# soon-yau/upgpt

Hardware: AMD Instinct MI355X
Metric: 256x256 images/sec, 50-step DDIM, bs=8/GPU; UNet MFMA util % (higher is better)
Workload: dtype f16; 1 GPU; BASELINE configs[1]: bs=8/GPU, 256x256 px (latent 4x32x32), 50-step DDIM eta=0, text-only cond [B,87,768], UNet(bbox.yaml) + VAE decode, EMA weights, no CFG; batch_per_gpu=8, ddim_steps=50, batches_in_flight_per_gpu=4, lane_hw_queues=measured, parallelism=replica-dp1, one all-gather of images per batch

## Files before the change

include/upk.h:

```cpp
#ifndef UPK_H_
#define UPK_H_

#include <stddef.h>
#include <stdint.h>

#ifdef __cplusplus
extern "C" {
#endif

#define UPK_VERSION 100

#define UPK_OK 0
#define UPK_EINVAL (-1)
#define UPK_ESHAPE (-2)
#define UPK_EWORKSPACE (-3)
#define UPK_EHIP (-4)
#define UPK_ENODEV (-5)

typedef struct upk_ctx upk_ctx;
typedef void* upk_stream;

int upk_version(void);
int upk_create(upk_ctx** out, int device);
int upk_destroy(upk_ctx* ctx);
// ... 121 lines not shown
  const float* vec;
  float ln_eps;
  int32_t ln_dim;
  void* t0;
  int32_t ld_t0;
  void* qk;
  int32_t ld_qk;
  void* vt;
  int32_t vt_ld;
  int32_t hw, rows_per_wg;
  const float* gn_part;
  const float* gn_gamma;
  const float* gn_beta;
  int32_t gn_nblk, gn_ld, gn_groups;
  float gn_eps;
} upk_hblock_desc;
int upk_head_block_f16(upk_ctx* ctx, const upk_hblock_desc* d, upk_stream stream);
int upk_head_block_supported(upk_ctx* ctx, const upk_hblock_desc* d);

int upk_gemm_f16(upk_ctx* ctx, const void* a, int lda, int m, int k, const void* w_packed,
                 int n_out, int n_pad, const float* bias, const void* residual, int ld_res,
                 void* y, int ldy, int flags, upk_stream stream);

int upk_conv_autotune(upk_ctx* ctx, const upk_conv_desc* d, upk_stream stream, int reps, int* best_cfg,
                      int* best_splitk, float* best_us, float* default_us);

int upk_conv_override(upk_ctx* ctx, int cfg, int splitk);
int upk_conv_num_configs(void);
const char* upk_conv_config_name(int cfg);

int upk_attention_f16(upk_ctx* ctx, const void* q, int ldq, long long q_batch_stride,
                      const void* k, int ldk, long long k_batch_stride, const void* vt, int vt_ld,
                      void* out, int ldo, long long o_batch_stride, int batch, int heads, int n_q,
                      int n_kv, int d, float scale, upk_stream stream);

int upk_attention_causal_f16(upk_ctx* ctx, const void* q, int ldq, long long q_batch_stride,
                             const void* k, int ldk, long long k_batch_stride, const void* vt, int vt_ld,
                             void* out, int ldo, long long o_batch_stride, int batch, int heads, int n,
                             int d, float scale, upk_stream stream);

int upk_attention_qproj_f16(upk_ctx* ctx, const void* x, int ldx, long long xbs, int cq, int ln_dim, float ln_eps,
                            const void* wq, const float* wq_colsum, const float* wq_bias, const void* k, int ldk,
                            long long kbs, const void* vt, int vt_ld, void* out, int ldo, long long obs, int batch,
                            int heads, int n_q, int n_kv, int d, float scale, upk_stream stream);

int upk_embed_tokens_f16(upk_ctx* ctx, const int32_t* ids, const void* tok_emb, const void* pos_emb, int rows,
                         int seq, int dim, int vocab, void* out, int ld_out, upk_stream stream);

int upk_gather_rows_f16(upk_ctx* ctx, const void* x, int ldx, const int32_t* idx, int n, int n_src, int dim,
// ... 105 lines not shown
```

upgpt_amd/_lib.py:

```python
import contextlib
import ctypes as C
import os
import threading

import torch
from ._check import require

_HERE = os.path.dirname(os.path.abspath(__file__))
LIB_PATH = os.environ.get("UPK_LIB") or os.path.join(_HERE, "libupk.so")

SYMBOLS = [
    "upk_version", "upk_create", "upk_destroy", "upk_last_error", "upk_set_workspace", "upk_num_cus",
    "upk_pack_weight_f16", "upk_packed_weight_bytes", "upk_conv2d_nhwc_f16", "upk_gemm_f16",
    "upk_conv_autotune", "upk_conv_override", "upk_conv_num_configs", "upk_conv_config_name", "upk_conv_gn_fused",
    "upk_conv_ln_rows",
    "upk_geglu_mlp_f16", "upk_geglu_mlp_supported", "upk_cross_block_f16", "upk_cross_block_supported", "upk_head_block_f16", "upk_head_block_supported",
    "upk_attention_f16", "upk_groupnorm_nhwc_f16", "upk_groupnorm_stats_nhwc_f16", "upk_groupnorm_chunks", "upk_groupnorm_apply_nhwc_f16", "upk_groupnorm_finalize_f32", "upk_groupnorm_ws_bytes",
    "upk_layernorm_f16", "upk_timestep_embed_f16",
    "upk_nchw_f32_to_nhwc_f16", "upk_nhwc_f16_to_nchw_f32", "upk_f32_to_f16", "upk_ddim_step_f32",
    "upk_ddim_step_cfg_f32", "upk_ddim_step_edit_f32", "upk_plms_step_f32", "upk_ddpm_step_f32", "upk_attention_causal_f16", "upk_attention_qproj_f16", "upk_embed_tokens_f16",
    "upk_patchify_nchw_f32_f16", "upk_vit_assemble_f16", "upk_gather_rows_f16",
    "upk_image_finish_u8", "upk_ssim_ws_bytes", "upk_ssim_u8",
    "upk_lpips_input_f16", "upk_relu_pool_nhwc_f16", "upk_lpips_ws_bytes", "upk_lpips_layer_f16",
    "upk_advance_step", "upk_step_autoadvance", "upk_kernel_launches", "upk_graph_begin", "upk_graph_end", "upk_graph_launch", "upk_graph_destroy",
    "upk_prof_enable", "upk_prof_collect",
    "upk_stream_create_cumask", "upk_stream_destroy", "upk_probe_placement", "upk_probe_clock",
]

F_SILU, F_GEGLU, F_OUT_F32, F_OUT_NCHW_F32, F_UPSAMPLE2X, F_PAD_ASYM = 0x1, 0x2, 0x4, 0x8, 0x10, 0x20
DDPM_X0, DDPM_CLIP = 0x1, 0x2
LAYOUT_NCHW, LAYOUT_NHWC = 0, 1
FINISH_SAMPLE, FINISH_INPUT, FINISH_DENORM = 0, 1, 2
# ... 53 lines not shown
        ("ln_eps", C.c_float), ("ln_dim", C.c_int32),
        ("k_ctx", C.c_void_p), ("ldk", C.c_int32), ("n_kv", C.c_int32),
        ("vt_ctx", C.c_void_p), ("vt_ld", C.c_int32), ("scale", C.c_float),
        ("y", C.c_void_p), ("ldy", C.c_int32), ("hw", C.c_int32), ("rows_per_wg", C.c_int32),
    ]


class HblockDesc(C.Structure):
    _fields_ = [
        ("x", C.c_void_p), ("ldx", C.c_int32), ("m", C.c_int32), ("c", C.c_int32), ("heads", C.c_int32), ("d", C.c_int32),
        ("w_in", C.c_void_p), ("w_qkv", C.c_void_p), ("vec", C.c_void_p), ("ln_eps", C.c_float), ("ln_dim", C.c_int32),
        ("t0", C.c_void_p), ("ld_t0", C.c_int32), ("qk", C.c_void_p), ("ld_qk", C.c_int32),
        ("vt", C.c_void_p), ("vt_ld", C.c_int32), ("hw", C.c_int32), ("rows_per_wg", C.c_int32),
        ("gn_part", C.c_void_p), ("gn_gamma", C.c_void_p), ("gn_beta", C.c_void_p),
        ("gn_nblk", C.c_int32), ("gn_ld", C.c_int32), ("gn_groups", C.c_int32), ("gn_eps", C.c_float),
    ]


_lib = None
_lib_lock = threading.Lock()


def load_library(path=None):
    global _lib
    with _lib_lock:
        if _lib is not None and path is None:
            return _lib
        p = path or LIB_PATH
        if not os.path.exists(p):
            raise RuntimeError(
# ... 14 lines not shown
            "upk_gemm_f16": (C.c_int, [vp, vp, i32, i32, i32, vp, i32, i32, vp, vp, i32, vp, i32, i32, vp]),
            "upk_conv_autotune": (C.c_int, [vp, C.POINTER(ConvDesc), vp, i32, C.POINTER(C.c_int), C.POINTER(C.c_int),
                                            C.POINTER(C.c_float), C.POINTER(C.c_float)]),
            "upk_conv_override": (C.c_int, [vp, i32, i32]),
            "upk_conv_num_configs": (C.c_int, []),
            "upk_conv_config_name": (C.c_char_p, [i32]),
            "upk_conv_ln_rows": (C.c_int, [vp, C.POINTER(ConvDesc), C.POINTER(C.c_int)]),
            "upk_geglu_mlp_f16": (C.c_int, [vp, C.POINTER(MlpDesc), vp]),
            "upk_geglu_mlp_supported": (C.c_int, [vp, C.POINTER(MlpDesc)]),
            "upk_cross_block_f16": (C.c_int, [vp, C.POINTER(XblockDesc), vp]),
            "upk_cross_block_supported": (C.c_int, [vp, C.POINTER(XblockDesc)]),
            "upk_head_block_f16": (C.c_int, [vp, C.POINTER(HblockDesc), vp]),
            "upk_head_block_supported": (C.c_int, [vp, C.POINTER(HblockDesc)]),
            "upk_attention_f16": (C.c_int, [vp, vp, i32, i64, vp, i32, i64, vp, i32, vp, i32, i64,
                                            i32, i32, i32, i32, i32, f32, vp]),
            "upk_attention_causal_f16": (C.c_int, [vp, vp, i32, i64, vp, i32, i64, vp, i32, vp, i32, i64,
                                                   i32, i32, i32, i32, f32, vp]),
            "upk_attention_qproj_f16": (C.c_int, [vp, vp, i32, i64, i32, i32, f32, vp, vp, vp, vp, i32, i64, vp, i32, vp,
                                                  i32, i64, i32, i32, i32, i32, i32, f32, vp]),
            "upk_embed_tokens_f16": (C.c_int, [vp, vp, vp, vp, i32, i32, i32, i32, vp, i32, vp]),
            "upk_gather_rows_f16": (C.c_int, [vp, vp, i32, vp, i32, i32, i32, vp, i32, vp]),
            "upk_patchify_nchw_f32_f16": (C.c_int, [vp, vp, i32, i32, i32, i32, i32, vp, i32, vp]),
            "upk_vit_assemble_f16": (C.c_int, [vp, vp, i32, vp, vp, i32, i32, i32, vp, i32, vp]),
            "upk_groupnorm_nhwc_f16": (C.c_int, [vp, vp, i32, i32, vp, i32, i32, i32, i32, i32, vp, vp,
                                                 f32, i32, vp, i32, vp, vp]),
            "upk_groupnorm_stats_nhwc_f16": (C.c_int, [vp, vp, i32, i32, vp, i32, i32, i32, i32, i32, vp, vp]),
            "upk_groupnorm_chunks": (C.c_int, [i32]),
            "upk_groupnorm_apply_nhwc_f16": (C.c_int, [vp, vp, i32, i32, vp, i32, i32, i32, i32, i32, vp, vp,
                                                       f32, i32, vp, i32, vp, i32, i32, i32, vp, i32, i32, vp]),
            "upk_conv_gn_fused": (C.c_int, [vp, C.POINTER(ConvDesc), C.POINTER(C.c_int), C.POINTER(C.c_int)]),
# ... 351 lines not shown
```

upgpt_amd/csrc/attention.hip:

```cpp
#include <stdlib.h>

#include "common.h"

namespace {

struct AttnArgs {
  const f16* q;
  const f16* k;
  const f16* vt;
  f16* o;
  int ldq, ldk, vt_ld, ldo;
  long qbs, kbs, obs;
  int heads, nq, nkv;
  float scale_log2;
  int causal;
};

__device__ __forceinline__ float raw_exp2(float x) { return __builtin_amdgcn_exp2f(x); }
__device__ __forceinline__ float max_over_key_groups(float x) {
  unsigned u = __float_as_uint(x);
  const auto a = __builtin_amdgcn_permlane32_swap(u, u, false, false);
  u = __float_as_uint(fmaxf(__uint_as_float(a[0]), __uint_as_float(a[1])));
  const auto b = __builtin_amdgcn_permlane16_swap(u, u, false, false);
  return fmaxf(__uint_as_float(b[0]), __uint_as_float(b[1]));
}
__device__ __forceinline__ float sum_over_key_groups(float x) {
  unsigned u = __float_as_uint(x);
  const auto a = __builtin_amdgcn_permlane32_swap(u, u, false, false);
  u = __float_as_uint(__uint_as_float(a[0]) + __uint_as_float(a[1]));
  const auto b = __builtin_amdgcn_permlane16_swap(u, u, false, false);
// ... 279 lines not shown
    if (!q_ok[u]) continue;
    f16* orow = a.o + b * a.obs + (long)(q0 + u * 16 + c) * a.ldo + h * D + g * 4;
#pragma unroll
    for (int i = 0; i < DT; ++i) {
      f16x4 ov;
#pragma unroll
      for (int r = 0; r < 4; ++r) ov[r] = (f16)(o[u][i][r] * inv);
      *(f16x4*)(orow + i * 16) = ov;
    }
  }
}

constexpr int ATT_VROW = 72;
__device__ __forceinline__ int att_swz(int row, int chunk) { return chunk ^ ((-(row >> 2)) & 3); }

template <int D, int QT>
__global__ __launch_bounds__(256) void attn_lds_kernel(const AttnArgs a) {
  constexpr int KD = D / 32;
  constexpr int DT = D / 16;
  __shared__ __attribute__((aligned(16))) f16 sk[2][KD * 64 * 32];
  __shared__ __attribute__((aligned(16))) f16 sv[2][D * ATT_VROW];
  const int tid = threadIdx.x;
  const int lane = tid & 63, wave = tid >> 6;
  const int g = lane >> 4, c = lane & 15;
  const int bh = blockIdx.x;
#ifndef UPK_NO_XCD_SAMPLE
  const int nb_ = gridDim.x / a.heads;
  const int b = bh % nb_;
  const int h = bh / nb_;
#else
  const int b = bh / a.heads;
// ... 4 lines not shown

  bool q_ok[QT];
  f16x8 qf[QT][KD];
  f32x4 o[QT][DT];
  float mrun[QT];
  f32x4 lsum[QT];
#pragma unroll
  for (int u = 0; u < QT; ++u) {
    const int qi = q0 + u * 16 + c;
    q_ok[u] = qi < a.nq;
    const f16* qrow = a.q + b * a.qbs + (long)(q_ok[u] ? qi : 0) * a.ldq + h * D + g * 8;
#pragma unroll
    for (int kd = 0; kd < KD; ++kd) qf[u][kd] = q_ok[u] ? *(const f16x8*)(qrow + kd * 32) : zero8;
#pragma unroll
    for (int i = 0; i < DT; ++i) o[u][i] = (f32x4){0.f, 0.f, 0.f, 0.f};
    mrun[u] = -INFINITY;
    lsum[u] = (f32x4){0.f, 0.f, 0.f, 0.f};
  }
  const f16* ksrc = a.k + b * a.kbs + (long)(tid >> 2) * a.ldk + h * D + (tid & 3) * 8;
  const f16* vsrc = a.vt + ((long)(b * a.heads + h) * D + (tid >> 3)) * a.vt_ld + (tid & 7) * 8;
  const int kdst = (tid >> 2) * 32 + att_swz(tid >> 2, tid & 3) * 8;
  const int vdst = (tid >> 3) * ATT_VROW + (tid & 7) * 8;
  f16x8 kreg[KD], vreg[KD];
  auto fetch = [&](int kb) {
#pragma unroll
    for (int it = 0; it < KD; ++it) {
      kreg[it] = *(const f16x8*)(ksrc + (long)kb * a.ldk + it * 32);
      vreg[it] = *(const f16x8*)(vsrc + (long)it * 32 * a.vt_ld + kb);
    }
  };
  auto stash = [&](int buf) {
// ... 4 lines not shown
    }
  };
  const int ntiles = a.nkv >> 6;
  fetch(0);
  stash(0);
  __syncthreads();
  const float cs = a.scale_log2;
  const int kfrag = c * 32 + att_swz(c, g) * 8;
  for (int t = 0; t < ntiles; ++t) {
    const int buf = t & 1;
    if (t + 1 < ntiles) fetch((t + 1) << 6);
    f32x4 sc[QT][4];
#pragma unroll
    for (int tt = 0; tt < 4; ++tt)
#pragma unroll
      for (int u = 0; u < QT; ++u) sc[u][tt] = (f32x4){0.f, 0.f, 0.f, 0.f};
#pragma unroll
    for (int kd = 0; kd < KD; ++kd)
#pragma unroll
      for (int tt = 0; tt < 4; ++tt) {
        const f16x8 kf = *(const f16x8*)(&sk[buf][(kd * 64 + tt * 16) * 32 + kfrag]);
#pragma unroll
        for (int u = 0; u < QT; ++u) sc[u][tt] = __builtin_amdgcn_mfma_f32_16x16x32_f16(kf, qf[u][kd], sc[u][tt], 0, 0, 0);
      }
    f16x8 pf[QT][2];
#pragma unroll
    for (int u = 0; u < QT; ++u) {
      float mx = -INFINITY;
#pragma unroll
      for (int tt = 0; tt < 4; ++tt)
        mx = fmaxf(mx, fmaxf(fmaxf(sc[u][tt][0], sc[u][tt][1]), fmaxf(sc[u][tt][2], sc[u][tt][3])));
      mx = max_over_key_groups(mx);
      const float mnew = fmaxf(mrun[u], mx);
      if (__builtin_amdgcn_ballot_w64(mnew != mrun[u]) != 0) {
        const float alpha = raw_exp2((mrun[u] - mnew) * cs);
        lsum[u] *= alpha;
#pragma unroll
        for (int i = 0; i < DT; ++i) o[u][i] *= alpha;
      }
      mrun[u] = mnew;
      const float mc = -mnew * cs;
#pragma unroll
      for (int tt = 0; tt < 4; ++tt)
#pragma unroll
        for (int r = 0; r < 4; ++r) pf[u][tt >> 1][(tt & 1) * 4 + r] = (f16)raw_exp2(fmaf(sc[u][tt][r], cs, mc));
    }
#pragma unroll
    for (int j = 0; j < 2; ++j)
#pragma unroll
      for (int u = 0; u < QT; ++u) lsum[u] = __builtin_amdgcn_mfma_f32_16x16x32_f16(ATT_ONES, pf[u][j], lsum[u], 0, 0, 0);
#pragma unroll
    for (int i = 0; i < DT; ++i)
#pragma unroll
      for (int j = 0; j < 2; ++j) {
        const f16* vr = &sv[buf][(i * 16 + c) * ATT_VROW + 32 * j + 4 * g];
        const f16x4 va = *(const f16x4*)vr, vb = *(const f16x4*)(vr + 16);
        const f16x8 vf = {va[0], va[1], va[2], va[3], vb[0], vb[1], vb[2], vb[3]};
#pragma unroll
        for (int u = 0; u < QT; ++u) o[u][i] = __builtin_amdgcn_mfma_f32_16x16x32_f16(vf, pf[u][j], o[u][i], 0, 0, 0);
      }
// ... 117 lines not shown
  }
  if (!q_ok) return;
  const float inv = 1.0f / lsum[0];
  f16* orow = a.o + b * a.obs + (long)(q0 + c) * a.ldo + g * 4;
#pragma unroll
  for (int i = 0; i < DT; ++i) {
    f16x4 ov;
#pragma unroll
    for (int r = 0; r < 4; ++r) ov[r] = (f16)(o[i][r] * inv);
    *(f16x4*)(orow + i * 16) = ov;
  }
}

static int attention_impl(upk_ctx* ctx, const void* q, int ldq, long long qbs, const void* k, int ldk, long long kbs,
                          const void* vt, int vt_ld, void* out, int ldo, long long obs, int batch, int heads, int n_q,
                          int n_kv, int d, float scale, int causal, upk_stream stream_) {
  if (!ctx) return UPK_EINVAL;
  if (!q || !k || !vt || !out) return upk_fail(ctx, UPK_EINVAL, "attention: null pointer");
  if (batch <= 0 || heads <= 0 || n_q <= 0 || n_kv <= 0) return upk_fail(ctx, UPK_EINVAL, "attention: empty");
  if ((ldq & 7) || (ldk & 7) || (vt_ld & 3) || (ldo & 3) || vt_ld < ((n_kv + 31) & ~31))
    return upk_fail(ctx, UPK_EINVAL, "attention: ldq/ldk %% 8, vt_ld %% 4 and vt_ld >= round_up(n_kv,32) required");
  hipStream_t stream = (hipStream_t)stream_;
  AttnArgs a;
  a.q = (const f16*)q;
  a.k = (const f16*)k;
  a.vt = (const f16*)vt;
  a.o = (f16*)out;
  a.ldq = ldq;
  a.ldk = ldk;
  a.vt_ld = vt_ld;
  a.ldo = ldo;
  a.qbs = qbs;
  a.kbs = kbs;
  a.obs = obs;
  a.heads = heads;
  a.nq = n_q;
  a.nkv = n_kv;
  a.scale_log2 = scale * 1.4426950408889634f;
  a.causal = causal;
  if (causal && n_q != n_kv) return upk_fail(ctx, UPK_EINVAL, "attention: causal needs n_q == n_kv");
  static const int qt_env = getenv("UPK_ATTN_QT") ? atoi(getenv("UPK_ATTN_QT")) : 0;
  const int qt = qt_env ? qt_env : ((d <= 128 && (long)((n_q + 127) / 128) * batch * heads >= 4L * ctx->num_cus) ? 2 : 1);
  dim3 grid(batch * heads, (n_q + 64 * qt - 1) / (64 * qt)), block(256);
  upk_prof_scope prof(ctx, UPK_CLS_ATTN, stream);
  static const bool lds_off = getenv("UPK_ATTN_DIRECT") != nullptr;
  if (!lds_off && !causal && (d == 32 || d == 64) && n_kv >= 256 && (n_kv & 63) == 0 && (vt_ld & 7) == 0) {
    if (d == 32) {
      if (qt == 2) hipLaunchKernelGGL((attn_lds_kernel<32, 2>), grid, block, 0, stream, a);
      else hipLaunchKernelGGL((attn_lds_kernel<32, 1>), grid, block, 0, stream, a);
    } else {
      if (qt == 2) hipLaunchKernelGGL((attn_lds_kernel<64, 2>), grid, block, 0, stream, a);
      else hipLaunchKernelGGL((attn_lds_kernel<64, 1>), grid, block, 0, stream, a);
    }
    return upk_check_launch(ctx, "attention_lds");
  }
  {
    const int wpb = attn_waves_per_block(ctx, batch * heads, n_q, d <= 128 ? qt : 1);
    if (d <= 128) {
      grid = dim3(batch * heads, (n_q + 16 * qt * wpb - 1) / (16 * qt * wpb));
      block = dim3(64 * wpb);
    }
  }
#define UPK_ATTN(D_, QR_)                                                                         \
  if (qt == 2)                                                                                    \
    hipLaunchKernelGGL((attn_kernel<D_, QR_, (D_ <= 128 ? 2 : 1)>), grid, block, 0, stream, a);  \
  else                                                                                            \
    hipLaunchKernelGGL((attn_kernel<D_, QR_, 1>), grid, block, 0, stream, a);
  switch (d) {
// ... 18 lines not shown
      const dim3 g2(batch * heads, (n_q + 16 * wpb - 1) / (16 * wpb)), b2(64 * wpb);
      if (d == 256) hipLaunchKernelGGL((attn_kernel<256, 1, 1>), g2, b2, 0, stream, a);
      else hipLaunchKernelGGL((attn_kernel<512, 0, 1>), g2, b2, 0, stream, a);
      break;
    }
    default: return upk_fail(ctx, UPK_ESHAPE, "attention: head dim %d not in {32,64,128,256,512}", d);
  }
#undef UPK_ATTN
  return upk_check_launch(ctx, "attention");
}

extern "C" int upk_attention_f16(upk_ctx* ctx, const void* q, int ldq, long long qbs, const void* k, int ldk,
                                 long long kbs, const void* vt, int vt_ld, void* out, int ldo, long long obs,
                                 int batch, int heads, int n_q, int n_kv, int d, float scale, upk_stream stream) {
  return attention_impl(ctx, q, ldq, qbs, k, ldk, kbs, vt, vt_ld, out, ldo, obs, batch, heads, n_q, n_kv, d, scale, 0,
                        stream);
}

extern "C" int upk_attention_causal_f16(upk_ctx* ctx, const void* q, int ldq, long long qbs, const void* k, int ldk,
                                        long long kbs, const void* vt, int vt_ld, void* out, int ldo, long long obs,
                                        int batch, int heads, int n, int d, float scale, upk_stream stream) {
  return attention_impl(ctx, q, ldq, qbs, k, ldk, kbs, vt, vt_ld, out, ldo, obs, batch, heads, n, n, d, scale, 1, stream);
}

extern "C" int upk_attention_qproj_f16(upk_ctx* ctx, const void* x, int ldx, long long xbs, int cq, int ln_dim,
                                       float ln_eps, const void* wq, const float* wq_colsum, const float* wq_bias,
                                       const void* k, int ldk, long long kbs, const void* vt, int vt_ld, void* out,
                                       int ldo, long long obs, int batch, int heads, int n_q, int n_kv, int d,
                                       float scale, upk_stream stream_) {
  if (!ctx) return UPK_EINVAL;
  if (!x || !wq || !wq_colsum || !wq_bias || !k || !vt || !out) return upk_fail(ctx, UPK_EINVAL, "attention_qproj: null pointer");
  if (batch <= 0 || heads <= 0 || n_q <= 0 || n_kv <= 0) return upk_fail(ctx, UPK_EINVAL, "attention_qproj: empty");
  if ((ldx & 7) || (ldk & 7) || (vt_ld & 3) || (ldo & 3) || vt_ld < ((n_kv + 31) & ~31))
    return upk_fail(ctx, UPK_EINVAL, "attention_qproj: ldx/ldk %% 8, vt_ld %% 4 and vt_ld >= round_up(n_kv,32) required");
  if ((d != 32 && d != 64) || cq <= 0 || cq % 224 || ln_dim <= 0 || ln_dim > cq || ldx < cq)
    return upk_fail(ctx, UPK_ESHAPE, "attention_qproj: head dim %d / %d input channels outside {32,64} / 224*n", d, cq);
  hipStream_t stream = (hipStream_t)stream_;
// ... 2 lines not shown
  a.k = (const f16*)k;
  a.vt = (const f16*)vt;
  a.o = (f16*)out;
  a.ldq = 0;
  a.ldk = ldk;
  a.vt_ld = vt_ld;
  a.ldo = ldo;
  a.qbs = 0;
  a.kbs = kbs;
  a.obs = obs;
  a.heads = heads;
  a.nq = n_q;
  a.nkv = n_kv;
  a.scale_log2 = scale * 1.4426950408889634f;
  a.causal = 0;
  QProj p;
  p.x = (const f16*)x;
  p.w = (const f16*)wq;
  p.u = wq_colsum;
  p.bias = wq_bias;
  p.xbs = xbs;
  p.ldx = ldx;
  p.cq = cq;
  p.ln_dim = ln_dim;
  p.eps = ln_eps;
  upk_prof_scope prof(ctx, UPK_CLS_ATTN, stream);
  const int qt = d == 32 ? 2 : 1;
  const int wpb = attn_waves_per_block(ctx, batch * heads, n_q, qt);
  const dim3 grid((n_q + 16 * qt * wpb - 1) / (16 * qt * wpb), batch * heads), block(64 * wpb);
  if (d == 32) hipLaunchKernelGGL((attn_qproj_kernel<32, 2>), grid, block, 0, stream, a, p);
// ... 4 lines not shown
```

upgpt_amd/csrc/xblock.hip:

```cpp
#include "igemm_common.h"

namespace upkd {
namespace {

constexpr int XB_NW = 8;
constexpr int XB_KEYS = 96;

struct XbArgs {
  const f16* a1;
  const f16* t0;
  const f16* w1;
  const f16* wq;
  const f16* w3;
  const f16* kc;
  const f16* vt;
  const f16* zero;
  const float* vec;
  f16* y;
  int lda, ldt0, ldy, ldk, vt_ld, M, hw, nkv, vec_pieces;
  float ln_inv_dim, ln_eps, scale_log2;
  unsigned long long* dbg;
};
#define XB_PIN(v) asm volatile("" ::"s"(v))

// ... 329 lines not shown
#undef STAMP
}


struct HbArgs {
  const f16* x;
  const f16* w1;
  const f16* w2;
  const f16* zero;
  const float* vec;
  f16* t0;
  f16* qk;
  f16* vt;
  int ldx, ldt0, ldqk, vt_ld, M, hw, vec_pieces;
  float ln_inv_dim, ln_eps;
  const float* gn_part;
  const float* gn_gamma;
  const float* gn_beta;
  int gn_nblk, gn_ld, gn_cpg;
  float gn_eps;
  unsigned long long* dbg;
};

template <int MI, int C32, int DP, bool GNF>
__global__ __launch_bounds__(512) void hblock_kernel(const HbArgs s) {
  constexpr int NW = XB_NW, BM = MI * 16;
  constexpr int C = C32 * 32, HD = NW * DP, N2 = 3 * HD;
  static_assert(C32 % 7 == 0, "C = 7 waves x NI1 fragments");
  constexpr int NI1 = C32 * 2 / 7;
  constexpr int NIQ = DP / 16;
// ... 182 lines not shown
#pragma unroll
    for (int i = 0; i < MI; ++i)
#pragma unroll
      for (int j = 0; j < NIQ; ++j) acc[i][j] = (f32x4){0.f, 0.f, 0.f, 0.f};
    static_assert(C32 == PF, "one ring block per pass");
    if (p < 2) xb_block<MI, NIQ, PF, BM, true>(acc, ring2, wb2 + (size_t)(p + 1) * HD * 64, ks2, loff, (const char*)tT + la);
    else xb_block<MI, NIQ, PF, BM, false>(acc, ring2, wb2, ks2, loff, (const char*)tT + la);
#pragma unroll
    for (int i = 0; i < MI; ++i) {
      const f32x2 mr = *(const f32x2*)(st + 2 * (i * 16 + lc));
      const int m = m0 + i * 16 + lc;
      const bool ok = m < s.M;
#pragma unroll
      for (int j = 0; j < NIQ; ++j) {
        const int n = p * HD + colq + j * 16 + lg * 4;
        const f32x4 v = (acc[i][j] - mr[0] * *(const f32x4*)(bl_u2 + n)) * mr[1] + *(const f32x4*)(bl_b2 + n);
        if (p < 2) {
          f16x4 o;
#pragma unroll
          for (int k = 0; k < 4; ++k) o[k] = (f16)v[k];
          if (ok) *(f16x4*)(s.qk + (unsigned)m * (unsigned)s.ldqk + n) = o;
        } else if (ok) {
          f16* dst = s.vt + ((long)(b * NW + wave) * DP + j * 16 + lg * 4) * s.vt_ld + tok0 + i * 16 + lc;
#pragma unroll
          for (int k = 0; k < 4; ++k) dst[(unsigned)k * (unsigned)s.vt_ld] = (f16)v[k];
        }
      }
    }
    STAMP(6 + p);
  }
#ifdef UPK_TIMELINE
// ... 86 lines not shown
  if (!d->x || !d->w_in || !d->w_qkv || !d->vec || !d->t0 || !d->qk || !d->vt)
    return upk_fail(ctx, UPK_EINVAL, "head_block: null operand");
  if (!upk_head_block_supported(ctx, d))
    return upk_fail(ctx, UPK_ESHAPE, "head_block: shape outside the fused kernel's domain (c=%d d=%d heads=%d)", d->c, d->d,
                    d->heads);
  hipStream_t stream = (hipStream_t)stream_;
  HbArgs s;
  memset(&s, 0, sizeof(s));
  s.x = (const f16*)d->x, s.w1 = (const f16*)d->w_in, s.w2 = (const f16*)d->w_qkv, s.zero = (const f16*)ctx->zero_page;
  s.vec = d->vec, s.t0 = (f16*)d->t0, s.qk = (f16*)d->qk, s.vt = (f16*)d->vt;
  s.ldx = d->ldx, s.ldt0 = d->ld_t0, s.ldqk = d->ld_qk, s.vt_ld = d->vt_ld, s.M = d->m, s.hw = d->hw;
  const int hd = d->heads * d->d;
  s.vec_pieces = (d->c + 6 * hd + 255) / 256;
  s.ln_inv_dim = 1.0f / (float)(d->ln_dim > 0 ? d->ln_dim : d->c);
  s.ln_eps = d->ln_eps;
#ifdef UPK_TIMELINE
  s.dbg = getenv("UPK_XB_TL") ? (unsigned long long*)((char*)ctx->ws + ctx->ws_bytes - 4096) : nullptr;
#endif
  const int bm = d->rows_per_wg > 0 ? d->rows_per_wg : 32;
  const bool gnf = d->gn_part != nullptr;
  if (gnf) {
    if (!d->gn_gamma || !d->gn_beta || d->gn_groups <= 0 || d->c % d->gn_groups || d->gn_groups > UPK_GN_GROUPS_MAX ||
        d->gn_nblk <= 0 || d->gn_nblk > UPK_GN_MAX_CHUNKS || d->gn_ld < d->c)
      return upk_fail(ctx, UPK_EINVAL, "head_block: bad GroupNorm operands (groups=%d nblk=%d ld=%d)", d->gn_groups,
                      d->gn_nblk, d->gn_ld);
    s.gn_part = d->gn_part, s.gn_gamma = d->gn_gamma, s.gn_beta = d->gn_beta;
    s.gn_nblk = d->gn_nblk, s.gn_ld = d->gn_ld, s.gn_cpg = d->c / d->gn_groups, s.gn_eps = d->gn_eps;
  }
  void (*fn)(const HbArgs) = bm == 32 ? (gnf ? hblock_kernel<2, 7, 32, true> : hblock_kernel<2, 7, 32, false>)
                                      : (gnf ? hblock_kernel<1, 7, 32, true> : hblock_kernel<1, 7, 32, false>);
// ... 9 lines not shown
```

upgpt_amd/emitter.py:

```python
import ctypes as C
import os

import torch

from . import _lib as L
from . import knobs as K
from ._check import require
from .packing import PW, Packer, _rup, head_pad
from .tuning import TUNE_CACHE, TUNE_CACHE_LANES


class Act:
    __slots__ = ("t", "B", "H", "W", "C", "gn_src", "ln_src")

    def __init__(self, t, B, H, W, C):
        self.t, self.B, self.H, self.W, self.C = t, B, H, W, C
        self.ln_src = None
        self.gn_src = None

    @property
    def ld(self):
        return self.t.shape[-1]

    @property
# ... 431 lines not shown
        P.igemm_flops += 2 * M * (2 * pw1.n_out * C_ + pw2.n_real * (pw1.n_out + C_))
        P.flops[-1] = 2 * M * (2 * pw1.n_out * C_ + pw2.n_real * (pw1.n_out + C_))
        return out

    def head_block_ok(self, x, t, heads, dp, qk, vt_ld):
        if K.HBLOCK == "0" or (t + ".hblock.vec") not in self.pk.w or x.C % 32:
            return False
        rows = K.XB_ROWS or 32
        d = L.HblockDesc()
        d.ldx, d.m, d.c, d.heads, d.d = x.C, x.M, x.C, heads, dp
        d.ld_t0, d.ld_qk, d.vt_ld, d.hw, d.rows_per_wg = x.C, qk.ld, vt_ld, x.H * x.W, rows
        if not self.lib.upk_head_block_supported(self.hctx, C.byref(d)):
            return False
        return K.HBLOCK == "1" or x.M // rows >= self.ctx.num_cus

    def head_block(self, P, x, n, t, heads, dp, qk, vt, vt_ld, gn):
        w = self.pk.w
        vec = w[t + ".hblock.vec"]
        gamma, beta, eps, ws = gn
        M, C_ = x.M, x.C
        hw = x.H * x.W
        rows = K.XB_ROWS or 32
        pi, qkv = w[n + ".proj_in"], w[t + ".attn1.qkv_ln"]
        armed = self._arm_gn_sources([x]) if K.HBLOCK_GN else None
        if armed is None:
            xn = self.groupnorm(P, x, gamma, beta, eps, False, ws)
        else:
            xn = Act(self.alloc(M, C_), x.B, x.H, x.W, C_)
        d = L.HblockDesc()
        d.x, d.ldx, d.m, d.c, d.heads, d.d = xn.t.data_ptr(), xn.ld, M, C_, heads, dp
        d.w_in, d.w_qkv, d.vec = pi.w.data_ptr(), qkv.w.data_ptr(), vec.data_ptr()
        d.ln_eps, d.ln_dim = 1e-5, C_
        d.qk, d.ld_qk, d.vt, d.vt_ld = qk.t.data_ptr(), qk.ld, vt.data_ptr(), vt_ld
        d.hw, d.rows_per_wg = hw, rows
        require(self.lib.upk_head_block_supported(self.hctx, C.byref(d)), "head_block: unsupported shape", RuntimeError)
        t0 = Act(self.alloc(M, C_), x.B, x.H, x.W, C_)
        d.t0, d.ld_t0 = t0.t.data_ptr(), t0.ld
        fn, h, chk = self.lib.upk_head_block_f16, self.hctx, self._chk
        label = "hblock M%d C%d d%d rows%d" % (M, C_, dp, rows)
        if armed is None:
            P.add(lambda s: chk(fn(h, C.byref(d), s)), d, xn, pi, qkv, vec, t0, qk, vt, cls="igemm_k1", label=label)
        else:
            fused_fn, apply_fn = self.lib.upk_conv_gn_fused, self.lib.upk_groupnorm_apply_nhwc_f16
            fin_fn, gn_fn = self.lib.upk_groupnorm_finalize_f32, self.lib.upk_groupnorm_nhwc_f16
            a = (x.t.data_ptr(), x.C, x.ld, None, 0, 0, x.B, hw, 32, gamma.data_ptr(), beta.data_ptr(), float(eps), 0,
                 xn.t.data_ptr(), xn.ld)
            src, sws = armed[0]
            mine = None
            if K.GN_REDUCE_APPLY and not isinstance(src, Emitter.GnProvider) and not src.gno_y:
# ... 54 lines not shown
        if not self.lib.upk_cross_block_supported(self.hctx, C.byref(d)):
            return None
        if K.XBLOCK == "auto" and M // rows < self.ctx.num_cus:
            return None
        out = Act(self.alloc(M, C_), t0.B, t0.H, t0.W, C_)
        d.y, d.ldy = out.t.data_ptr(), out.ld
        fn, h, chk = self.lib.upk_cross_block_f16, self.hctx, self._chk
        P.add(lambda s: chk(fn(h, C.byref(d), s)), d, a1, t0, o1, o2, ql, vec, kc, vtc, out, cls="igemm_k1",
              label="xblock M%d C%d d%d rows%d" % (M, C_, dp, rows))
        fl = 2 * M * (o1.k_real * o1.n_real + ql.k_real * ql.n_real + o2.k_real * o2.n_real)
        fl += 4 * M * heads * self.n_ctx * (ql.n_real // heads)
        P.igemm_flops += fl
        P.flops[-1] = fl
        return out

    def attention(self, P, q, ldq, qbs, k, ldk, kbs, vt, vt_ld, out, ldo, obs, B, heads, nq, nkv, dp, scale):
        fn, h, chk = self.lib.upk_attention_f16, self.hctx, self._chk
        a = (q.data_ptr(), ldq, qbs, k.data_ptr(), ldk, kbs, vt.data_ptr(), vt_ld, out.data_ptr(), ldo, obs, B, heads,
             nq, nkv, dp, float(scale))
        P.add(lambda s: chk(fn(h, *a, s)), q, k, vt, out, cls="attention",
              label="attn B%d h%d nq%d nkv%d d%d" % (B, heads, nq, nkv, dp))
```

upgpt_amd/engine.py:

```python
import ctypes as C
import os

import torch

from . import _lib as L
from . import knobs as K
from ._check import require
from .arch import UNetArch, VAEArch
from .emitter import Act, Emitter, Program
from .packing import (PW, PackedUNet, PackedVAEDecoder, PackedVAEEncoder, PackedVGG16, Packer, _rup,
                      geglu_rows_map, head_pad, pad_rows_map, qproj_pack, vgg16_convs)
from .tuning import TUNE_CACHE, TuneCache


class UNetPlan(Emitter):

    def __init__(self, ctx, packed: PackedUNet, B, H, W, n_ctx, rows, mode):
        super().__init__(ctx)
        require(mode in ("forward", "sampler"), "UNetPlan mode must be 'forward' or 'sampler'", ValueError)
        self.pk, self.arch = packed, packed.arch
        self.B, self.H, self.W, self.n_ctx, self.rows, self.mode = B, H, W, n_ctx, rows, mode
        a = self.arch
        mc, te = a.model_channels, a.time_embed_dim
        self.cin_pad = _rup(a.in_channels, 32)
# ... 65 lines not shown
            sk = x
        return self.conv(P, hh, w[n + ".out_layers.3"], residual=sk, gn=gn2, gn_stats=True)

    def _st(self, P, Lr, x):
        w, v = self.pk.w, self.pk.v
        n = Lr.name
        t = n + ".transformer_blocks.0"
        B, HW, M = x.B, x.H * x.W, x.M
        heads, dh = Lr.heads, Lr.dhead
        dp = head_pad(dh)
        hd = heads * dp
        scale = dh ** -0.5
        qk = Act(self.alloc(M, 2 * hd), B, x.H, x.W, 2 * hd)
        vt_ld = _rup(HW, 32)
        vt = self.alloc(B, heads, dp, vt_ld, zero=True)
        t0 = None
        if self.head_block_ok(x, t, heads, dp, qk, vt_ld):
            t0 = self.head_block(P, x, n, t, heads, dp, qk, vt, vt_ld, (*v[n + ".norm"], 1e-6, self.gn_ws))
        if t0 is None:
            t0 = self.conv(P, x, w[n + ".proj_in"], gn=(*v[n + ".norm"], 1e-6, False, self.gn_ws))
            self.ln_linear(P, t0, t + ".attn1.qkv", t + ".norm1", out=qk,
                           vt=dict(t=vt, heads=heads, dhead=dp, ld=vt_ld, tokens=HW, **{"from": 2 * hd}))
        a1 = Act(self.alloc(M, hd), B, x.H, x.W, hd)
        self.attention(P, qk.t, 2 * hd, HW * 2 * hd, qk.t[:, hd:], 2 * hd, HW * 2 * hd, vt, vt_ld, a1.t, hd, HW * hd,
                       B, heads, HW, HW, dp, scale)
        P.attn_flops += 4 * B * heads * HW * HW * dh
        kc, vtc, cld = self.kv[n]
        t2 = self.cross_block(P, a1, t0, t, kc, vtc, cld, heads, dp, scale)
        if t2 is not None:
            return self._st_ff(P, Lr, x, t2)
        t1 = self.conv(P, a1, w[t + ".attn1.to_out"], residual=t0)
        a2 = Act(self.alloc(M, hd), B, x.H, x.W, hd)
        if (K.QPROJ_FUSE and (t + ".attn2.qproj") in w and t1.C == t1.ld and dp == 32
                and B * heads * ((HW + 31) // 32) >= 2048):
            wq, wu, wb = w[t + ".attn2.qproj"]
            fn, hh, chk = self.lib.upk_attention_qproj_f16, self.hctx, self._chk
            qa = (t1.t.data_ptr(), t1.ld, HW * t1.ld, t1.C, t1.C, 1e-5, wq.data_ptr(), wu.data_ptr(), wb.data_ptr(),
                  kc.t.data_ptr(), hd, self.n_ctx * hd, vtc.data_ptr(), cld, a2.t.data_ptr(), hd, HW * hd, B, heads, HW,
                  self.n_ctx, dp, float(scale))
            P.add(lambda s: chk(fn(hh, *qa, s)), t1, wq, wu, wb, kc, vtc, a2, cls="attention",
# ... 399 lines not shown
```

Measured before the change: 97.59 images/s.

## Fold softmax scale into Q projection and use lazy max rescaling in attention

```diff
diff --git a/include/upk.h b/include/upk.h
--- a/include/upk.h
+++ b/include/upk.h
@@ -159,6 +159,7 @@
   const float* gn_beta;
   int32_t gn_nblk, gn_ld, gn_groups;
   float gn_eps;
+  float q_scale;
 } upk_hblock_desc;
 int upk_head_block_f16(upk_ctx* ctx, const upk_hblock_desc* d, upk_stream stream);
 int upk_head_block_supported(upk_ctx* ctx, const upk_hblock_desc* d);
@@ -178,6 +179,11 @@
                       const void* k, int ldk, long long k_batch_stride, const void* vt, int vt_ld,
                       void* out, int ldo, long long o_batch_stride, int batch, int heads, int n_q,
                       int n_kv, int d, float scale, upk_stream stream);
+#define UPK_ATTN_Q_PRESCALED 0x1u
+int upk_attention_ex_f16(upk_ctx* ctx, const void* q, int ldq, long long q_batch_stride,
+                         const void* k, int ldk, long long k_batch_stride, const void* vt, int vt_ld,
+                         void* out, int ldo, long long o_batch_stride, int batch, int heads, int n_q,
+                         int n_kv, int d, float scale, unsigned flags, upk_stream stream);
 
 int upk_attention_causal_f16(upk_ctx* ctx, const void* q, int ldq, long long q_batch_stride,
                              const void* k, int ldk, long long k_batch_stride, const void* vt, int vt_ld,
diff --git a/upgpt_amd/_lib.py b/upgpt_amd/_lib.py
--- a/upgpt_amd/_lib.py
+++ b/upgpt_amd/_lib.py
@@ -15,7 +15,7 @@
     "upk_conv_autotune", "upk_conv_override", "upk_conv_num_configs", "upk_conv_config_name", "upk_conv_gn_fused",
     "upk_conv_ln_rows",
     "upk_geglu_mlp_f16", "upk_geglu_mlp_supported", "upk_cross_block_f16", "upk_cross_block_supported", "upk_head_block_f16", "upk_head_block_supported",
-    "upk_attention_f16", "upk_groupnorm_nhwc_f16", "upk_groupnorm_stats_nhwc_f16", "upk_groupnorm_chunks", "upk_groupnorm_apply_nhwc_f16", "upk_groupnorm_finalize_f32", "upk_groupnorm_ws_bytes",
+    "upk_attention_f16", "upk_attention_ex_f16", "upk_groupnorm_nhwc_f16", "upk_groupnorm_stats_nhwc_f16", "upk_groupnorm_chunks", "upk_groupnorm_apply_nhwc_f16", "upk_groupnorm_finalize_f32", "upk_groupnorm_ws_bytes",
     "upk_layernorm_f16", "upk_timestep_embed_f16",
     "upk_nchw_f32_to_nhwc_f16", "upk_nhwc_f16_to_nchw_f32", "upk_f32_to_f16", "upk_ddim_step_f32",
     "upk_ddim_step_cfg_f32", "upk_ddim_step_edit_f32", "upk_plms_step_f32", "upk_ddpm_step_f32", "upk_attention_causal_f16", "upk_attention_qproj_f16", "upk_embed_tokens_f16",
@@ -99,6 +99,7 @@
         ("vt", C.c_void_p), ("vt_ld", C.c_int32), ("hw", C.c_int32), ("rows_per_wg", C.c_int32),
         ("gn_part", C.c_void_p), ("gn_gamma", C.c_void_p), ("gn_beta", C.c_void_p),
         ("gn_nblk", C.c_int32), ("gn_ld", C.c_int32), ("gn_groups", C.c_int32), ("gn_eps", C.c_float),
+        ("q_scale", C.c_float),
     ]
 
 
@@ -143,6 +144,8 @@
             "upk_head_block_supported": (C.c_int, [vp, C.POINTER(HblockDesc)]),
             "upk_attention_f16": (C.c_int, [vp, vp, i32, i64, vp, i32, i64, vp, i32, vp, i32, i64,
                                             i32, i32, i32, i32, i32, f32, vp]),
+            "upk_attention_ex_f16": (C.c_int, [vp, vp, i32, i64, vp, i32, i64, vp, i32, vp, i32, i64,
+                                               i32, i32, i32, i32, i32, f32, C.c_uint32, vp]),
             "upk_attention_causal_f16": (C.c_int, [vp, vp, i32, i64, vp, i32, i64, vp, i32, vp, i32, i64,
                                                    i32, i32, i32, i32, f32, vp]),
             "upk_attention_qproj_f16": (C.c_int, [vp, vp, i32, i64, i32, i32, f32, vp, vp, vp, vp, i32, i64, vp, i32, vp,
diff --git a/upgpt_amd/csrc/attention.hip b/upgpt_amd/csrc/attention.hip
--- a/upgpt_amd/csrc/attention.hip
+++ b/upgpt_amd/csrc/attention.hip
@@ -14,6 +14,7 @@
   int heads, nq, nkv;
   float scale_log2;
   int causal;
+  int q_scaled;
 };
 
 __device__ __forceinline__ float raw_exp2(float x) { return __builtin_amdgcn_exp2f(x); }
@@ -323,7 +324,7 @@
 constexpr int ATT_VROW = 72;
 __device__ __forceinline__ int att_swz(int row, int chunk) { return chunk ^ ((-(row >> 2)) & 3); }
 
-template <int D, int QT>
+template <int D, int QT, bool QS>
 __global__ __launch_bounds__(256) void attn_lds_kernel(const AttnArgs a) {
   constexpr int KD = D / 32;
   constexpr int DT = D / 16;
@@ -358,7 +359,7 @@
     for (int kd = 0; kd < KD; ++kd) qf[u][kd] = q_ok[u] ? *(const f16x8*)(qrow + kd * 32) : zero8;
 #pragma unroll
     for (int i = 0; i < DT; ++i) o[u][i] = (f32x4){0.f, 0.f, 0.f, 0.f};
-    mrun[u] = -INFINITY;
+    mrun[u] = 0.f;
     lsum[u] = (f32x4){0.f, 0.f, 0.f, 0.f};
   }
   const f16* ksrc = a.k + b * a.kbs + (long)(tid >> 2) * a.ldk + h * D + (tid & 3) * 8;
@@ -393,7 +394,10 @@
 #pragma unroll
     for (int tt = 0; tt < 4; ++tt)
 #pragma unroll
-      for (int u = 0; u < QT; ++u) sc[u][tt] = (f32x4){0.f, 0.f, 0.f, 0.f};
+      for (int u = 0; u < QT; ++u) {
+        const float m0 = QS ? -mrun[u] : 0.f;
+        sc[u][tt] = (f32x4){m0, m0, m0, m0};
+      }
 #pragma unroll
     for (int kd = 0; kd < KD; ++kd)
 #pragma unroll
@@ -405,24 +409,38 @@
     f16x8 pf[QT][2];
 #pragma unroll
     for (int u = 0; u < QT; ++u) {
-      float mx = -INFINITY;
+      if (!QS) {
+#pragma unroll
+        for (int tt = 0; tt < 4; ++tt)
+#pragma unroll
+          for (int r = 0; r < 4; ++r) sc[u][tt][r] = fmaf(sc[u][tt][r], cs, -mrun[u]);
+      }
+      float pos = 0.f;
 #pragma unroll
       for (int tt = 0; tt < 4; ++tt)
-        mx = fmaxf(mx, fmaxf(fmaxf(sc[u][tt][0], sc[u][tt][1]), fmaxf(sc[u][tt][2], sc[u][tt][3])));
-      mx = max_over_key_groups(mx);
-      const float mnew = fmaxf(mrun[u], mx);
-      if (__builtin_amdgcn_ballot_w64(mnew != mrun[u]) != 0) {
-        const float alpha = raw_exp2((mrun[u] - mnew) * cs);
-        lsum[u] *= alpha;
-#pragma unroll
-        for (int i = 0; i < DT; ++i) o[u][i] *= alpha;
-      }
-      mrun[u] = mnew;
-      const float mc = -mnew * cs;
+        pos = fmaxf(fmaxf(fmaxf(pos, sc[u][tt][0]), sc[u][tt][1]), fmaxf(sc[u][tt][2], sc[u][tt][3]));
+      if (t == 0 || __builtin_amdgcn_ballot_w64(pos > 0.f) != 0) {
+        float mx = -INFINITY;
+#pragma unroll
+        for (int tt = 0; tt < 4; ++tt)
+          mx = fmaxf(mx, fmaxf(fmaxf(sc[u][tt][0], sc[u][tt][1]), fmaxf(sc[u][tt][2], sc[u][tt][3])));
+        mx = max_over_key_groups(mx);
+        float d = mx;
+        if (t != 0) {
+          d = fmaxf(mx, 0.f);
+          const float alpha = raw_exp2(-d);
+          lsum[u] *= alpha;
+#pragma unroll
+          for (int i = 0; i < DT; ++i) o[u][i] *= alpha;
+        }
+        mrun[u] += d;
+#pragma unroll
+        for (int tt = 0; tt < 4; ++tt) sc[u][tt] -= d;
+      }
 #pragma unroll
       for (int tt = 0; tt < 4; ++tt)
 #pragma unroll
-        for (int r = 0; r < 4; ++r) pf[u][tt >> 1][(tt & 1) * 4 + r] = (f16)raw_exp2(fmaf(sc[u][tt][r], cs, mc));
+        for (int r = 0; r < 4; ++r) pf[u][tt >> 1][(tt & 1) * 4 + r] = (f16)raw_exp2(sc[u][tt][r]);
     }
 #pragma unroll
     for (int j = 0; j < 2; ++j)
@@ -570,8 +588,9 @@
 
 static int attention_impl(upk_ctx* ctx, const void* q, int ldq, long long qbs, const void* k, int ldk, long long kbs,
                           const void* vt, int vt_ld, void* out, int ldo, long long obs, int batch, int heads, int n_q,
-                          int n_kv, int d, float scale, int causal, upk_stream stream_) {
+                          int n_kv, int d, float scale, int causal, unsigned flags, upk_stream stream_) {
   if (!ctx) return UPK_EINVAL;
+  if (flags & ~(unsigned)UPK_ATTN_Q_PRESCALED) return upk_fail(ctx, UPK_EINVAL, "attention: unknown flags 0x%x", flags);
   if (!q || !k || !vt || !out) return upk_fail(ctx, UPK_EINVAL, "attention: null pointer");
   if (batch <= 0 || heads <= 0 || n_q <= 0 || n_kv <= 0) return upk_fail(ctx, UPK_EINVAL, "attention: empty");
   if ((ldq & 7) || (ldk & 7) || (vt_ld & 3) || (ldo & 3) || vt_ld < ((n_kv + 31) & ~31))
@@ -592,7 +611,8 @@
   a.heads = heads;
   a.nq = n_q;
   a.nkv = n_kv;
-  a.scale_log2 = scale * 1.4426950408889634f;
+  a.q_scaled = (flags & UPK_ATTN_Q_PRESCALED) ? 1 : 0;
+  a.scale_log2 = a.q_scaled ? 1.0f : scale * 1.4426950408889634f;
   a.causal = causal;
   if (causal && n_q != n_kv) return upk_fail(ctx, UPK_EINVAL, "attention: causal needs n_q == n_kv");
   static const int qt_env = getenv("UPK_ATTN_QT") ? atoi(getenv("UPK_ATTN_QT")) : 0;
@@ -601,13 +621,15 @@
   upk_prof_scope prof(ctx, UPK_CLS_ATTN, stream);
   static const bool lds_off = getenv("UPK_ATTN_DIRECT") != nullptr;
   if (!lds_off && !causal && (d == 32 || d == 64) && n_kv >= 256 && (n_kv & 63) == 0 && (vt_ld & 7) == 0) {
+#define UPK_ATTN_LDS(D_, QT_)                                                                     \
+  if (a.q_scaled) hipLaunchKernelGGL((attn_lds_kernel<D_, QT_, true>), grid, block, 0, stream, a); \
+  else hipLaunchKernelGGL((attn_lds_kernel<D_, QT_, false>), grid, block, 0, stream, a);
     if (d == 32) {
-      if (qt == 2) hipLaunchKernelGGL((attn_lds_kernel<32, 2>), grid, block, 0, stream, a);
-      else hipLaunchKernelGGL((attn_lds_kernel<32, 1>), grid, block, 0, stream, a);
+      if (qt == 2) { UPK_ATTN_LDS(32, 2) } else { UPK_ATTN_LDS(32, 1) }
     } else {
-      if (qt == 2) hipLaunchKernelGGL((attn_lds_kernel<64, 2>), grid, block, 0, stream, a);
-      else hipLaunchKernelGGL((attn_lds_kernel<64, 1>), grid, block, 0, stream, a);
-    }
+      if (qt == 2) { UPK_ATTN_LDS(64, 2) } else { UPK_ATTN_LDS(64, 1) }
+    }
+#undef UPK_ATTN_LDS
     return upk_check_launch(ctx, "attention_lds");
   }
   {
@@ -656,13 +678,21 @@
                                  long long kbs, const void* vt, int vt_ld, void* out, int ldo, long long obs,
                                  int batch, int heads, int n_q, int n_kv, int d, float scale, upk_stream stream) {
   return attention_impl(ctx, q, ldq, qbs, k, ldk, kbs, vt, vt_ld, out, ldo, obs, batch, heads, n_q, n_kv, d, scale, 0,
-                        stream);
+                        0, stream);
+}
+
+extern "C" int upk_attention_ex_f16(upk_ctx* ctx, const void* q, int ldq, long long qbs, const void* k, int ldk,
+                                    long long kbs, const void* vt, int vt_ld, void* out, int ldo, long long obs,
+                                    int batch, int heads, int n_q, int n_kv, int d, float scale, unsigned flags,
+                                    upk_stream stream) {
+  return attention_impl(ctx, q, ldq, qbs, k, ldk, kbs, vt, vt_ld, out, ldo, obs, batch, heads, n_q, n_kv, d, scale, 0,
+                        flags, stream);
 }
 
 extern "C" int upk_attention_causal_f16(upk_ctx* ctx, const void* q, int ldq, long long qbs, const void* k, int ldk,
                                         long long kbs, const void* vt, int vt_ld, void* out, int ldo, long long obs,
                                         int batch, int heads, int n, int d, float scale, upk_stream stream) {
-  return attention_impl(ctx, q, ldq, qbs, k, ldk, kbs, vt, vt_ld, out, ldo, obs, batch, heads, n, n, d, scale, 1, stream);
+  return attention_impl(ctx, q, ldq, qbs, k, ldk, kbs, vt, vt_ld, out, ldo, obs, batch, heads, n, n, d, scale, 1, 0, stream);
 }
 
 extern "C" int upk_attention_qproj_f16(upk_ctx* ctx, const void* x, int ldx, long long xbs, int cq, int ln_dim,
@@ -695,6 +725,7 @@
   a.nkv = n_kv;
   a.scale_log2 = scale * 1.4426950408889634f;
   a.causal = 0;
+  a.q_scaled = 0;
   QProj p;
   p.x = (const f16*)x;
   p.w = (const f16*)wq;
diff --git a/upgpt_amd/csrc/xblock.hip b/upgpt_amd/csrc/xblock.hip
--- a/upgpt_amd/csrc/xblock.hip
+++ b/upgpt_amd/csrc/xblock.hip
@@ -367,6 +367,7 @@
   f16* vt;
   int ldx, ldt0, ldqk, vt_ld, M, hw, vec_pieces;
   float ln_inv_dim, ln_eps;
+  float q_scale;
   const float* gn_part;
   const float* gn_gamma;
   const float* gn_beta;
@@ -579,7 +580,8 @@
 #pragma unroll
       for (int j = 0; j < NIQ; ++j) {
         const int n = p * HD + colq + j * 16 + lg * 4;
-        const f32x4 v = (acc[i][j] - mr[0] * *(const f32x4*)(bl_u2 + n)) * mr[1] + *(const f32x4*)(bl_b2 + n);
+        f32x4 v = (acc[i][j] - mr[0] * *(const f32x4*)(bl_u2 + n)) * mr[1] + *(const f32x4*)(bl_b2 + n);
+        if (p == 0) v *= s.q_scale;
         if (p < 2) {
           f16x4 o;
 #pragma unroll
@@ -696,6 +698,7 @@
   s.vec_pieces = (d->c + 6 * hd + 255) / 256;
   s.ln_inv_dim = 1.0f / (float)(d->ln_dim > 0 ? d->ln_dim : d->c);
   s.ln_eps = d->ln_eps;
+  s.q_scale = d->q_scale != 0.f ? d->q_scale : 1.0f;
 #ifdef UPK_TIMELINE
   s.dbg = getenv("UPK_XB_TL") ? (unsigned long long*)((char*)ctx->ws + ctx->ws_bytes - 4096) : nullptr;
 #endif
diff --git a/upgpt_amd/emitter.py b/upgpt_amd/emitter.py
--- a/upgpt_amd/emitter.py
+++ b/upgpt_amd/emitter.py
@@ -469,7 +469,7 @@
             return False
         return K.HBLOCK == "1" or x.M // rows >= self.ctx.num_cus
 
-    def head_block(self, P, x, n, t, heads, dp, qk, vt, vt_ld, gn):
+    def head_block(self, P, x, n, t, heads, dp, qk, vt, vt_ld, gn, q_scale=0.0):
         w = self.pk.w
         vec = w[t + ".hblock.vec"]
         gamma, beta, eps, ws = gn
@@ -487,7 +487,7 @@
         d.w_in, d.w_qkv, d.vec = pi.w.data_ptr(), qkv.w.data_ptr(), vec.data_ptr()
         d.ln_eps, d.ln_dim = 1e-5, C_
         d.qk, d.ld_qk, d.vt, d.vt_ld = qk.t.data_ptr(), qk.ld, vt.data_ptr(), vt_ld
-        d.hw, d.rows_per_wg = hw, rows
+        d.hw, d.rows_per_wg, d.q_scale = hw, rows, float(q_scale)
         require(self.lib.upk_head_block_supported(self.hctx, C.byref(d)), "head_block: unsupported shape", RuntimeError)
         t0 = Act(self.alloc(M, C_), x.B, x.H, x.W, C_)
         d.t0, d.ld_t0 = t0.t.data_ptr(), t0.ld
@@ -572,9 +572,10 @@
         P.flops[-1] = fl
         return out
 
-    def attention(self, P, q, ldq, qbs, k, ldk, kbs, vt, vt_ld, out, ldo, obs, B, heads, nq, nkv, dp, scale):
-        fn, h, chk = self.lib.upk_attention_f16, self.hctx, self._chk
+    def attention(self, P, q, ldq, qbs, k, ldk, kbs, vt, vt_ld, out, ldo, obs, B, heads, nq, nkv, dp, scale,
+                  q_prescaled=False):
+        fn, h, chk = self.lib.upk_attention_ex_f16, self.hctx, self._chk
         a = (q.data_ptr(), ldq, qbs, k.data_ptr(), ldk, kbs, vt.data_ptr(), vt_ld, out.data_ptr(), ldo, obs, B, heads,
-             nq, nkv, dp, float(scale))
+             nq, nkv, dp, float(scale), 1 if q_prescaled else 0)
         P.add(lambda s: chk(fn(h, *a, s)), q, k, vt, out, cls="attention",
               label="attn B%d h%d nq%d nkv%d d%d" % (B, heads, nq, nkv, dp))
diff --git a/upgpt_amd/engine.py b/upgpt_amd/engine.py
--- a/upgpt_amd/engine.py
+++ b/upgpt_amd/engine.py
@@ -103,16 +103,18 @@
         qk = Act(self.alloc(M, 2 * hd), B, x.H, x.W, 2 * hd)
         vt_ld = _rup(HW, 32)
         vt = self.alloc(B, heads, dp, vt_ld, zero=True)
-        t0 = None
+        t0, q_pre = None, False
         if self.head_block_ok(x, t, heads, dp, qk, vt_ld):
-            t0 = self.head_block(P, x, n, t, heads, dp, qk, vt, vt_ld, (*v[n + ".norm"], 1e-6, self.gn_ws))
+            t0 = self.head_block(P, x, n, t, heads, dp, qk, vt, vt_ld, (*v[n + ".norm"], 1e-6, self.gn_ws),
+                                 q_scale=scale * 1.4426950408889634)
+            q_pre = True
         if t0 is None:
             t0 = self.conv(P, x, w[n + ".proj_in"], gn=(*v[n + ".norm"], 1e-6, False, self.gn_ws))
             self.ln_linear(P, t0, t + ".attn1.qkv", t + ".norm1", out=qk,
                            vt=dict(t=vt, heads=heads, dhead=dp, ld=vt_ld, tokens=HW, **{"from": 2 * hd}))
         a1 = Act(self.alloc(M, hd), B, x.H, x.W, hd)
         self.attention(P, qk.t, 2 * hd, HW * 2 * hd, qk.t[:, hd:], 2 * hd, HW * 2 * hd, vt, vt_ld, a1.t, hd, HW * hd,
-                       B, heads, HW, HW, dp, scale)
+                       B, heads, HW, HW, dp, scale, q_prescaled=q_pre)
         P.attn_flops += 4 * B * heads * HW * HW * dh
         kc, vtc, cld = self.kv[n]
         t2 = self.cross_block(P, a1, t0, t, kc, vtc, cld, heads, dp, scale)
```

Measured after the change: 96.75 images/s. About the same (-0.9%).
